# letao1991/EAD-GAN

Hardware: AMD Instinct MI355X
Metric: imgs/sec per G+D+E train step, CelebA 64x64 bs=128 (higher is better)
Workload: dtype bf16; 1 GPU; EAD-GAN CelebA 64x64x3 full train iteration (G adv + D + info/affine, 3 Adams), batch 128/GPU, hipGraph replay, data-parallel x1; per_gpu_batch=128, global_batch=128, parallelism=dp1

## Files before the change

### ead-gan_amd/csrc/img_conv.hip

```cpp

#include "eg_common.h"
#include "igemm_nt.h"

#ifndef EG_IMG_CONV_OCC
#define EG_IMG_CONV_OCC 3
#endif

struct ImgMfmaParams {
    const float* img[4];
    const float* gate[4];
    const void* wp;
    void* out;
    const float* bias;
    const float* sigma;
    int B, C, H, W;
    int act;
    float slope;
    int gate_act;
    float gate_slope;
    const void* stat_z;
    const float* stat_p[4];
    float* stat_out;
    int stat_act;
    float stat_slope;
};

constexpr int img_conv_occ(int N) { return N == 128 ? EG_IMG_CONV_OCC : (N == 64 ? 4 : 6); }
template <typename T, bool STAT, int N = 128>
__global__ __launch_bounds__(256, STAT ? 2 : img_conv_occ(N)) void conv_img_mfma_kernel(const ImgMfmaParams p, int ntiles) {
    static_assert(N == 128 || N == 64 || N == 32, "column tiles of 16, whole 64-byte chunks per pixel row");
    static_assert(!STAT || N == 128 || N == 64, "the statistics epilogue writes 2 N sums from 256 threads");
    constexpr int NJ = N / 16;
    constexpr int XS = 72, OS = N + 8;
    __shared__ __attribute__((aligned(16))) unsigned short s_in[4][6][XS];
    __shared__ __attribute__((aligned(16))) unsigned short s_out[4][16][OS];
    const int tid = threadIdx.x, lane = tid & 63, wave = tid >> 6;
    const int frow = lane & 15, fq = lane >> 4;
    const int OH = p.H >> 1, OW = p.W >> 1;
    const int gxn = OW >> 5, tpi = (OH >> 1) * gxn;
    const T* __restrict__ wp = reinterpret_cast<const T*>(p.wp);

    uint4 bf[2][NJ];
#pragma unroll
    for (int s = 0; s < 2; ++s)
#pragma unroll
        for (int j = 0; j < NJ; ++j) bf[s][j] = *reinterpret_cast<const uint4*>(wp + (size_t)(j * 16 + frow) * 64 + s * 32 + fq * 8);
    __shared__ __attribute__((aligned(16))) float s_bias[N];
    __shared__ __attribute__((aligned(16))) float s_red[STAT ? 4 * 2 * N : 4];
    if (tid < N) s_bias[tid] = p.bias ? p.bias[tid] : 0.f;
    __shared__ __attribute__((aligned(16))) float s_par[STAT ? 4 * N : 4];
    if constexpr (STAT) {
        if (tid < N) {
            const float mu = p.stat_p[0][tid], is = p.stat_p[1][tid], g = p.stat_p[2][tid], bb = p.stat_p[3][tid];
            const float P = __fmul_rn(g, is);
            s_par[tid] = mu; s_par[N + tid] = is; s_par[2 * N + tid] = P; s_par[3 * N + tid] = __fsub_rn(bb, __fmul_rn(mu, P));
        }
    }
    const EgGradFast sgf = eg_grad_fast(p.stat_act, p.stat_slope);
    const EgActFast af = eg_act_fast(p.act, p.slope);

    struct Slot { float4 v; float lo, hi; };
    auto fetch = [&](int tile, int e, Slot& sl) {
        sl.v = make_float4(0.f, 0.f, 0.f, 0.f); sl.lo = 0.f; sl.hi = 0.f;
        if (e >= 4 * 6 * 16 || tile >= ntiles) return;
        const int ib = tile / tpi, rem_t = tile - ib * tpi;
        const int tape = ib / p.B, b = ib - tape * p.B;
        const int gx = rem_t % gxn, oy0 = (rem_t / gxn) * 2;
        const int c = e / 96, rem = e - c * 96, r = rem >> 4, x4 = rem & 15;
        const int iy = 2 * oy0 - 1 + r, x0 = gx * 64;
        if (c >= p.C || iy < 0 || iy >= p.H) return;
        const size_t o = (((size_t)b * p.C + c) * p.H + iy) * p.W + x0 + x4 * 4;
        const float* __restrict__ img = p.img[tape];
        const float* __restrict__ gate = p.gate[tape];
        sl.v = *reinterpret_cast<const float4*>(img + o);
        if (x4 == 0 && x0 > 0) sl.lo = img[o - 1];
        if (x4 == 15 && x0 + 64 < p.W) sl.hi = img[o + 4];
        if (gate) {
            const float4 g = *reinterpret_cast<const float4*>(gate + o);
            sl.v.x *= eg_act_grad_from_out(g.x, p.gate_act, p.gate_slope); sl.v.y *= eg_act_grad_from_out(g.y, p.gate_act, p.gate_slope);
            sl.v.z *= eg_act_grad_from_out(g.z, p.gate_act, p.gate_slope); sl.v.w *= eg_act_grad_from_out(g.w, p.gate_act, p.gate_slope);
            if (x4 == 0 && x0 > 0) sl.lo *= eg_act_grad_from_out(gate[o - 1], p.gate_act, p.gate_slope);
            if (x4 == 15 && x0 + 64 < p.W) sl.hi *= eg_act_grad_from_out(gate[o + 4], p.gate_act, p.gate_slope);
        }
    };
    auto stage = [&](int e, const Slot& sl) {
        if (e >= 4 * 6 * 16) return;
        const int c = e / 96, rem = e - c * 96, r = rem >> 4, x4 = rem & 15;
        T h[4];
        Elt<T>::st(h + 0, sl.v.x); Elt<T>::st(h + 1, sl.v.y); Elt<T>::st(h + 2, sl.v.z); Elt<T>::st(h + 3, sl.v.w);
        unsigned short* row = &s_in[c][r][0];
        const unsigned short* hb = reinterpret_cast<const unsigned short*>(h);
        row[1 + x4 * 4] = hb[0];
        *reinterpret_cast<unsigned*>(row + 2 + x4 * 4) = (unsigned)hb[1] | ((unsigned)hb[2] << 16);
        row[4 + x4 * 4] = hb[3];
        if (x4 == 0) { T t; Elt<T>::st(&t, sl.lo); row[0] = *reinterpret_cast<const unsigned short*>(&t); }
        if (x4 == 15) { T t; Elt<T>::st(&t, sl.hi); row[65] = *reinterpret_cast<const unsigned short*>(&t); }
    };

    const int ry = wave >> 1, oxl = (wave & 1) * 16 + frow;
    const int r0 = 2 * ry + (fq & 1) * 2;
    auto ld8 = [&](int c, int r) {
        const unsigned* q = reinterpret_cast<const unsigned*>(&s_in[c][r][2 * oxl]);
        return make_uint2(q[0], q[1]);
    };
    T* __restrict__ out = reinterpret_cast<T*>(p.out);

    Slot s0, s1;
    int tile = blockIdx.x;
    fetch(tile, tid, s0); fetch(tile, tid + 256, s1);
    for (; tile < ntiles; tile += gridDim.x) {
        stage(tid, s0); stage(tid + 256, s1);
        __syncthreads();
        fetch(tile + gridDim.x, tid, s0); fetch(tile + gridDim.x, tid + 256, s1);
        const uint2 a00 = ld8(fq >> 1, r0), a01 = ld8(fq >> 1, r0 + 1);
        const uint2 a10 = ld8(2 + (fq >> 1), r0), a11 = ld8(2 + (fq >> 1), r0 + 1);
        const uint4 a0 = make_uint4(a00.x, a00.y, a01.x, a01.y), a1 = make_uint4(a10.x, a10.y, a11.x, a11.y);
        f32x4 acc[NJ];
#pragma unroll
        for (int j = 0; j < NJ; ++j) acc[j] = (f32x4){0.f, 0.f, 0.f, 0.f};
#pragma unroll
        for (int j = 0; j < NJ; ++j) mfma_step<T>(a0, bf[0][j], acc[j]);
#pragma unroll
        for (int j = 0; j < NJ; ++j) mfma_step<T>(a1, bf[1][j], acc[j]);
        const int ib = tile / tpi, rem_t = tile - ib * tpi;
        const int tape = ib / p.B;
        const int gx = rem_t % gxn, oy0 = (rem_t / gxn) * 2;
        const float inv_sigma = p.sigma ? 1.f / p.sigma[tape] : 1.f;
        const size_t pix0 = ((size_t)ib * OH + oy0 + ry) * OW + gx * 32 + (wave & 1) * 16;
#pragma unroll
        for (int j = 0; j < NJ; ++j) {
            T h[4];
            const float4 bv = *reinterpret_cast<const float4*>(&s_bias[j * 16 + fq * 4]);
            const float bj[4] = {bv.x, bv.y, bv.z, bv.w};
#pragma unroll
            for (int r = 0; r < 4; ++r) {
                float x = __fmul_rn(acc[j][r], inv_sigma);
                if (p.bias) x = __fadd_rn(x, bj[r]);
                x = af.special ? eg_act(x, p.act, p.slope) : eg_act_apply(x, af);
                Elt<T>::st(h + r, x);
            }
            if constexpr (STAT) {
                const uint2 zv = *reinterpret_cast<const uint2*>(reinterpret_cast<const T*>(p.stat_z) + (pix0 + frow) * N + j * 16 + fq * 4);
                const T* ze = reinterpret_cast<const T*>(&zv);
                float s1[4], s2[4];
                const int nb = j * 16 + fq * 4;
                const float4 vmu = *reinterpret_cast<const float4*>(&s_par[nb]), vis = *reinterpret_cast<const float4*>(&s_par[N + nb]);
                const float4 vp = *reinterpret_cast<const float4*>(&s_par[2 * N + nb]), vq = *reinterpret_cast<const float4*>(&s_par[3 * N + nb]);
                const float k_mu[4] = {vmu.x, vmu.y, vmu.z, vmu.w}, k_is[4] = {vis.x, vis.y, vis.z, vis.w};
                const float k_p[4] = {vp.x, vp.y, vp.z, vp.w}, k_q[4] = {vq.x, vq.y, vq.z, vq.w};
#pragma unroll
                for (int r = 0; r < 4; ++r) {
                    const float z = Elt<T>::ld(ze + r);
                    const float xh = (z - k_mu[r]) * k_is[r];
                    const float dy = Elt<T>::ld(h + r) * eg_grad_apply(fmaf(z, k_p[r], k_q[r]), sgf);
                    Elt<T>::st(h + r, dy);
                    s1[r] = dy;
                    s2[r] = dy * xh;
                }
#pragma unroll
                for (int r = 0; r < 4; ++r) {
                    s1[r] += eg_dpp<0xB1>(s1[r]); s1[r] += eg_dpp<0x4E>(s1[r]); s1[r] += eg_dpp<0x141>(s1[r]); s1[r] += eg_dpp<0x140>(s1[r]);
                    s2[r] += eg_dpp<0xB1>(s2[r]); s2[r] += eg_dpp<0x4E>(s2[r]); s2[r] += eg_dpp<0x141>(s2[r]); s2[r] += eg_dpp<0x140>(s2[r]);
                }
                if (frow == 0) {
                    *reinterpret_cast<float4*>(&s_red[(wave * 2 + 0) * N + j * 16 + fq * 4]) = make_float4(s1[0], s1[1], s1[2], s1[3]);
                    *reinterpret_cast<float4*>(&s_red[(wave * 2 + 1) * N + j * 16 + fq * 4]) = make_float4(s2[0], s2[1], s2[2], s2[3]);
                }
            }
            *reinterpret_cast<uint2*>(&s_out[wave][frow][j * 16 + fq * 4]) = *reinterpret_cast<const uint2*>(h);
        }
        __syncthreads();
        if constexpr (STAT) {
            if (tid < 2 * N) {
                const int which = tid / N, n = tid - which * N;
                const float t = ((s_red[(0 * 2 + which) * N + n] + s_red[(1 * 2 + which) * N + n]) + s_red[(2 * 2 + which) * N + n]) + s_red[(3 * 2 + which) * N + n];
                p.stat_out[((size_t)which * N + n) * ntiles + tile] = t;
            }
        }
        constexpr int CPR = N / 8, RPI = 64 / CPR;
#pragma unroll
        for (int it = 0; it < 16 / RPI; ++it) {
            const int row = it * RPI + lane / CPR, chunk = lane % CPR;
            const uint4 v = *reinterpret_cast<const uint4*>(&s_out[wave][row][chunk * 8]);
            *reinterpret_cast<uint4*>(out + (pix0 + row) * N + chunk * 8) = v;
        }
    }
}

extern "C" int eg_conv_img_mfma_stat_blocks(int B, int H, int W, int ntapes) { return (H / 4) * (W / 64) * B * ntapes; }

extern "C" int eg_conv_img_mfma_ok(int dtype, int C, int H, int W, int N, int k, int stride, int pad) {
    return dtype != EG_F32 && C >= 1 && C <= 4 && (N == 128 || N == 64 || N == 32) && k == 4 && stride == 2 && pad == 1 && H >= 4 && (H % 4) == 0 && (W % 64) == 0;
}

extern "C" int eg_conv_img_mfma_n(int dtype, const float* img0, const float* img1, const float* img2, const float* gate0, const float* gate1,
                                  const float* gate2, int ntapes, const void* wp, void* out, int B, int C, int H, int W, int N, const eg_epilogue* ep,
                                  int gate_act, float gate_slope, eg_stream_t s) {
    EG_REQUIRE(img0 && wp && out && ntapes >= 1 && ntapes <= 3 && B > 0, "eg_conv_img_mfma: bad argument");
    EG_REQUIRE(eg_conv_img_mfma_ok(dtype, C, H, W, N, 4, 2, 1), "eg_conv_img_mfma: 16-bit types, C <= 4, N = 32 / 64 / 128, H %% 4 == 0, W %% 64 == 0 only (use eg_im2col_img + eg_conv_fwd)");
    EG_REQUIRE((ntapes < 2 || img1) && (ntapes < 3 || img2), "eg_conv_img_mfma: one image pointer per tape");
    EG_REQUIRE(!ep || (!ep->mask && ep->out_mode == EG_OUT_NHWC && ep->bias_mod == 0 && (ep->stat_mode == EG_STAT_NONE || ep->stat_mode == EG_STAT_BN_BWD)),
               "eg_conv_img_mfma: unsupported epilogue field");
    const bool stat = ep && ep->stat_mode == EG_STAT_BN_BWD;
    EG_REQUIRE(!stat || N == 128 || N == 64, "eg_conv_img_mfma: EG_STAT_BN_BWD with 128 or 64 output channels only");
    EG_REQUIRE(!stat || (ep->stat_out && ep->stat_aux && ep->stat_p0 && ep->stat_p1 && ep->stat_p2 && ep->stat_p3), "eg_conv_img_mfma: EG_STAT_BN_BWD needs stat_out, stat_aux (z) and stat_p0..p3");
    ImgMfmaParams p;
    memset(&p, 0, sizeof(p));
    p.img[0] = img0; p.img[1] = img1; p.img[2] = img2;
    p.gate[0] = gate0; p.gate[1] = gate1; p.gate[2] = gate2;
    p.wp = wp; p.out = out; p.B = B; p.C = C; p.H = H; p.W = W;
    p.bias = ep ? ep->bias : nullptr;
    p.sigma = ep ? ep->sigma : nullptr;
    p.act = ep ? ep->act : EG_ACT_NONE;
    p.slope = ep ? ep->slope : 0.f;
    p.gate_act = gate_act; p.gate_slope = gate_slope;
    if (stat) {
        p.stat_z = ep->stat_aux; p.stat_out = ep->stat_out; p.stat_act = ep->stat_act; p.stat_slope = ep->stat_slope;
        p.stat_p[0] = ep->stat_p0; p.stat_p[1] = ep->stat_p1; p.stat_p[2] = ep->stat_p2; p.stat_p[3] = ep->stat_p3;
    }
    const int ntiles = (H / 4) * (W / 64) * B * ntapes;
    const int wgs_n = N == 128 ? 256 * EG_IMG_CONV_OCC : 256 * img_conv_occ(N);
    const dim3 grid(ntiles < wgs_n ? ntiles : wgs_n);
    if (stat) {
        const dim3 gs(ntiles < 512 ? ntiles : 512);
        if (N == 64) {
            if (dtype == EG_F16) hipLaunchKernelGGL((conv_img_mfma_kernel<f16_t, true, 64>), gs, dim3(256), 0, (hipStream_t)s, p, ntiles);
            else hipLaunchKernelGGL((conv_img_mfma_kernel<bf16_t, true, 64>), gs, dim3(256), 0, (hipStream_t)s, p, ntiles);
        } else if (dtype == EG_F16) hipLaunchKernelGGL((conv_img_mfma_kernel<f16_t, true>), gs, dim3(256), 0, (hipStream_t)s, p, ntiles);
        else hipLaunchKernelGGL((conv_img_mfma_kernel<bf16_t, true>), gs, dim3(256), 0, (hipStream_t)s, p, ntiles);
    } else if (N == 128) {
        if (dtype == EG_F16) hipLaunchKernelGGL((conv_img_mfma_kernel<f16_t, false>), grid, dim3(256), 0, (hipStream_t)s, p, ntiles);
        else hipLaunchKernelGGL((conv_img_mfma_kernel<bf16_t, false>), grid, dim3(256), 0, (hipStream_t)s, p, ntiles);
    } else if (N == 64) {
        if (dtype == EG_F16) hipLaunchKernelGGL((conv_img_mfma_kernel<f16_t, false, 64>), grid, dim3(256), 0, (hipStream_t)s, p, ntiles);
        else hipLaunchKernelGGL((conv_img_mfma_kernel<bf16_t, false, 64>), grid, dim3(256), 0, (hipStream_t)s, p, ntiles);
    } else {
        if (dtype == EG_F16) hipLaunchKernelGGL((conv_img_mfma_kernel<f16_t, false, 32>), grid, dim3(256), 0, (hipStream_t)s, p, ntiles);
        else hipLaunchKernelGGL((conv_img_mfma_kernel<bf16_t, false, 32>), grid, dim3(256), 0, (hipStream_t)s, p, ntiles);
    }
    EG_LAUNCH_CHECK();
    return 0;
}

extern "C" int eg_conv_img_mfma(int dtype, const float* img0, const float* img1, const float* img2, const float* gate0, const float* gate1,
                                const float* gate2, int ntapes, const void* wp, void* out, int B, int C, int H, int W, const eg_epilogue* ep,
                                int gate_act, float gate_slope, eg_stream_t s) {
    return eg_conv_img_mfma_n(dtype, img0, img1, img2, gate0, gate1, gate2, ntapes, wp, out, B, C, H, W, 128, ep, gate_act, gate_slope, s);
}

struct ImgTParams {
    const void* a;
    const void* wp;
    const float* bias;
    float* out;
    int B, C, Hin, Win;
    int act;
    float slope;
};

template <typename T, int R, int K = 128>
__global__ __launch_bounds__(256) void convt_img_mfma_kernel(const ImgTParams p) {
    constexpr int KS = K / 32;
    constexpr int WMAX = 32, NP = 56;
    __shared__ __attribute__((aligned(16))) unsigned short s_cols[(R + 2) * WMAX * NP];
    const int tid = threadIdx.x, lane = tid & 63, wave = tid >> 6;
    const int frow = lane & 15, fq = lane >> 4;
    const int nblk = p.Hin / R, b = blockIdx.x / nblk, r0 = (blockIdx.x % nblk) * R;
    const int ncol = 16 * p.C;
    const T* __restrict__ wp = reinterpret_cast<const T*>(p.wp);
    const T* __restrict__ a = reinterpret_cast<const T*>(p.a) + (size_t)b * p.Hin * p.Win * K;

    uint4 bf[KS][3];
#pragma unroll
    for (int s = 0; s < KS; ++s)
#pragma unroll
        for (int j = 0; j < 3; ++j) {
            const int n = j * 16 + frow;
            bf[s][j] = n < ncol ? *reinterpret_cast<const uint4*>(wp + (size_t)n * K + s * 32 + fq * 8) : make_uint4(0, 0, 0, 0);
        }
    const int npix = (R + 2) * p.Win, ngrp = npix / 16;
    auto fetch = [&](int g, uint4 (&af)[KS]) {
        const int pl = g * 16 + frow;
        const int iy = r0 - 1 + pl / p.Win, ix = pl % p.Win;
        const bool ok = g < ngrp && iy >= 0 && iy < p.Hin;
#pragma unroll
        for (int s = 0; s < KS; ++s)
            af[s] = ok ? *reinterpret_cast<const uint4*>(a + ((size_t)iy * p.Win + ix) * K + s * 32 + fq * 8) : make_uint4(0, 0, 0, 0);
    };
    auto compute = [&](int g, const uint4 (&af)[KS]) {
        const int pl = g * 16 + frow;
        f32x4 acc[3];
#pragma unroll
        for (int j = 0; j < 3; ++j) acc[j] = (f32x4){0.f, 0.f, 0.f, 0.f};
#pragma unroll
        for (int s = 0; s < KS; ++s)
#pragma unroll
            for (int j = 0; j < 3; ++j) mfma_step<T>(af[s], bf[s][j], acc[j]);
#pragma unroll
        for (int j = 0; j < 3; ++j) {
            T h[4];
#pragma unroll
            for (int r = 0; r < 4; ++r) Elt<T>::st(h + r, __fmul_rn(acc[j][r], 1.f));
            *reinterpret_cast<uint2*>(&s_cols[(size_t)pl * NP + j * 16 + fq * 4]) = *reinterpret_cast<const uint2*>(h);
        }
    };
    uint4 fa[KS], fb[KS];
    fetch(wave, fa);
    for (int g = wave; g < ngrp; g += 8) {
        fetch(g + 4, fb);
        compute(g, fa);
        if (g + 4 < ngrp) {
            fetch(g + 8, fa);
            compute(g + 4, fb);
        }
    }
    __syncthreads();
    const int OH = 2 * p.Hin, OW = 2 * p.Win;
    const T* __restrict__ cols = reinterpret_cast<const T*>(s_cols);
    for (int o = tid; o < 2 * R * OW; o += 256) {
        const int ox = o % OW, oy = 2 * r0 + o / OW;
        float acc[3];
#pragma unroll
        for (int c = 0; c < 3; ++c) acc[c] = (p.bias && c < p.C) ? p.bias[c] : 0.f;
        for (int kh = (oy + 1) & 1; kh < 4; kh += 2) {
            const int iy = (oy + 1 - kh) >> 1;
            if (iy < 0 || iy >= p.Hin) continue;
            for (int kw = (ox + 1) & 1; kw < 4; kw += 2) {
                const int ix = (ox + 1 - kw) >> 1;
                if (ix < 0 || ix >= p.Win) continue;
                const T* src = cols + (size_t)((iy - (r0 - 1)) * p.Win + ix) * NP + (kh * 4 + kw) * p.C;
#pragma unroll
                for (int c = 0; c < 3; ++c)
                    if (c < p.C) acc[c] += Elt<T>::ld(src + c);
            }
        }
#pragma unroll
        for (int c = 0; c < 3; ++c)
            if (c < p.C) p.out[(((size_t)b * p.C + c) * OH + oy) * OW + ox] = eg_act(acc[c], p.act, p.slope);
    }
}

extern "C" int eg_convt_img_mfma_ok(int dtype, int C, int Hin, int Win, int K, int k, int stride, int pad) {
    return dtype != EG_F32 && C >= 1 && C <= 3 && (K == 128 || K == 64) && k == 4 && stride == 2 && pad == 1 && Hin >= 16 && (Hin % 16) == 0 && (Win == 16 || Win == 32);
}

extern "C" int eg_convt_img_mfma_k(int dtype, const void* a, const void* wp, const float* bias, float* out, int B, int C, int Hin, int Win, int K, int act,
                                   float slope, eg_stream_t s) {
    EG_REQUIRE(a && wp && out && B > 0, "eg_convt_img_mfma: bad argument");
    EG_REQUIRE(eg_convt_img_mfma_ok(dtype, C, Hin, Win, K, 4, 2, 1), "eg_convt_img_mfma: 16-bit types, C <= 3, K = 64 / 128, Hin %% 16 == 0, Win 16 or 32 only (use eg_conv_fwd + eg_col2im_img)");
    ImgTParams p;
    memset(&p, 0, sizeof(p));
    p.a = a; p.wp = wp; p.bias = bias; p.out = out; p.B = B; p.C = C; p.Hin = Hin; p.Win = Win; p.act = act; p.slope = slope;
    hipStream_t st = (hipStream_t)s;
    if (K == 64) {
        const dim3 grid(B * (Hin / 8));
        if (dtype == EG_F16) hipLaunchKernelGGL((convt_img_mfma_kernel<f16_t, 8, 64>), grid, dim3(256), 0, st, p);
        else hipLaunchKernelGGL((convt_img_mfma_kernel<bf16_t, 8, 64>), grid, dim3(256), 0, st, p);
        EG_LAUNCH_CHECK();
        return 0;
    }
    const dim3 grid(B * (Hin / 8));
    if (dtype == EG_F16) hipLaunchKernelGGL((convt_img_mfma_kernel<f16_t, 8>), grid, dim3(256), 0, st, p);
    else hipLaunchKernelGGL((convt_img_mfma_kernel<bf16_t, 8>), grid, dim3(256), 0, st, p);
    EG_LAUNCH_CHECK();
    return 0;
}
extern "C" int eg_convt_img_mfma(int dtype, const void* a, const void* wp, const float* bias, float* out, int B, int C, int Hin, int Win, int act,
                                 float slope, eg_stream_t s) {
    return eg_convt_img_mfma_k(dtype, a, wp, bias, out, B, C, Hin, Win, 128, act, slope, s);
}

struct ImgWgradParams {
    const float* img[4];
    const void* P;
    float* slab;
    int B, C, ntiles;
};

template <typename T, int N>
__global__ __launch_bounds__(256) void wgrad_img_kernel(const ImgWgradParams p) {
    constexpr int H = 64, W = 64, OW = 32, XS = 72;
    constexpr int PP = N + 8, PX = 72;
    constexpr int NI = N / 16;
    __shared__ __attribute__((aligned(16))) unsigned short s_in[4][10][XS];
    __shared__ __attribute__((aligned(16))) unsigned short s_px[128 * PP + 128 * PX];
    unsigned short* s_p = s_px;
    unsigned short* s_x = s_px + 128 * PP;
    static_assert(4 * N * 16 * sizeof(float) <= (128 * PP + 128 * PX) * sizeof(unsigned short), "the reduction scratch lies over the operand tiles");
    float (*s_red)[N][16] = reinterpret_cast<float (*)[N][16]>(s_px);
    const int tid = threadIdx.x, lane = tid & 63, wave = tid >> 6;
    const int g = lane >> 4, li = lane & 15, q = li >> 2, pc = li & 3;
    const int kc = p.C * 16, nj = p.C;
    const T* __restrict__ P = reinterpret_cast<const T*>(p.P);
    for (int i = tid; i < 4 * 10 * XS; i += 256) (&s_in[0][0][0])[i] = 0;
    for (int i = tid; i < 128 * PX; i += 256) s_x[i] = 0;
    f32x4 acc[NI][4];
#pragma unroll
    for (int i = 0; i < NI; ++i)
#pragma unroll
        for (int j = 0; j < 4; ++j) acc[i][j] = (f32x4){0.f, 0.f, 0.f, 0.f};
    typedef __attribute__((address_space(3))) s16x4* lds_s16x4;
    auto tr2 = [&](const unsigned short* base, int pitch, int row, int blk) {
        const s16x4 lo = __builtin_amdgcn_ds_read_tr16_b64_v4i16((lds_s16x4)(base + (row + q) * pitch + blk * 16 + pc * 4));
        const s16x4 hi = __builtin_amdgcn_ds_read_tr16_b64_v4i16((lds_s16x4)(base + (row + 4 + q) * pitch + blk * 16 + pc * 4));
        return make_uint4(((uint32_t)(uint16_t)lo[0]) | ((uint32_t)(uint16_t)lo[1] << 16), ((uint32_t)(uint16_t)lo[2]) | ((uint32_t)(uint16_t)lo[3] << 16),
                          ((uint32_t)(uint16_t)hi[0]) | ((uint32_t)(uint16_t)hi[1] << 16), ((uint32_t)(uint16_t)hi[2]) | ((uint32_t)(uint16_t)hi[3] << 16));
    };
    for (int tile = blockIdx.x; tile < p.ntiles; tile += gridDim.x) {
        const int ib = tile >> 3, oy0 = (tile & 7) * 4;
        const int tape = ib / p.B, b = ib - tape * p.B;
        const float* __restrict__ img = p.img[tape] + (size_t)b * p.C * H * W;
        __syncthreads();
        for (int e = tid; e < p.C * 10 * 16; e += 256) {
            const int c = e / 160, rem = e - c * 160, r = rem >> 4, x4 = rem & 15;
            const int iy = 2 * oy0 - 1 + r;
            float4 v = make_float4(0.f, 0.f, 0.f, 0.f);
            if (iy >= 0 && iy < H) v = *reinterpret_cast<const float4*>(img + ((size_t)c * H + iy) * W + x4 * 4);
            T h[4];
            Elt<T>::st(h + 0, v.x); Elt<T>::st(h + 1, v.y); Elt<T>::st(h + 2, v.z); Elt<T>::st(h + 3, v.w);
            const unsigned short* hb = reinterpret_cast<const unsigned short*>(h);
            unsigned short* row = &s_in[c][r][1 + x4 * 4];
            row[0] = hb[0]; row[1] = hb[1]; row[2] = hb[2]; row[3] = hb[3];
        }
        const T* __restrict__ Pt = P + ((size_t)ib * 1024 + (size_t)oy0 * OW) * N;
        for (int e = tid; e < 128 * (N / 8); e += 256) {
            const int row = e / (N / 8), ch = e - row * (N / 8);
            *reinterpret_cast<uint4*>(&s_p[row * PP + ch * 8]) = *reinterpret_cast<const uint4*>(Pt + (size_t)row * N + ch * 8);
        }
        __syncthreads();
        for (int e = tid; e < 128 * kc; e += 256) {
            const int pix = e / kc, k = e - pix * kc;
            const int c = k >> 4, ky = (k >> 2) & 3, kx = k & 3;
            s_x[pix * PX + k] = s_in[c][2 * (pix >> 5) + ky][2 * (pix & 31) + kx];
        }
        __syncthreads();
        const int kb = wave * 32 + 8 * g;
        uint4 af[NI], bfr[4];
#pragma unroll
        for (int i = 0; i < NI; ++i) af[i] = tr2(s_p, PP, kb, i);
#pragma unroll
        for (int j = 0; j < 4; ++j)
            if (j < nj) bfr[j] = tr2(s_x, PX, kb, j);
#pragma unroll
        for (int i = 0; i < NI; ++i)
#pragma unroll
            for (int j = 0; j < 4; ++j)
                if (j < nj) {
                    if constexpr (std::is_same<T, f16_t>::value)
                        acc[i][j] = __builtin_amdgcn_mfma_f32_16x16x32_f16(__builtin_bit_cast(f16x8_t, af[i]), __builtin_bit_cast(f16x8_t, bfr[j]), acc[i][j], 0, 0, 0);
                    else
                        acc[i][j] = __builtin_amdgcn_mfma_f32_16x16x32_bf16(__builtin_bit_cast(bf16x8_t, af[i]), __builtin_bit_cast(bf16x8_t, bfr[j]), acc[i][j], 0, 0, 0);
                }
    }
    float* slab = p.slab + (size_t)blockIdx.x * N * kc;
    for (int j = 0; j < nj; ++j) {
        __syncthreads();
#pragma unroll
        for (int i = 0; i < NI; ++i)
#pragma unroll
            for (int r = 0; r < 4; ++r) {
                float v = 0.f;
#pragma unroll
                for (int jj = 0; jj < 4; ++jj)
                    if (jj == j) v = acc[i][jj][r];
                s_red[wave][i * 16 + g * 4 + r][li] = v;
            }
        __syncthreads();
        for (int e = tid; e < N * 16; e += 256) {
            const int n = e >> 4, k = e & 15;
            slab[(size_t)n * kc + j * 16 + k] = ((s_red[0][n][k] + s_red[1][n][k]) + s_red[2][n][k]) + s_red[3][n][k];
        }
    }
}

extern "C" int eg_wgrad_img_ok(int dtype, int C, int H, int W, int N, int k, int stride, int pad) {
    return dtype != EG_F32 && C >= 1 && C <= 4 && (N == 32 || N == 64 || N == 128) && k == 4 && stride == 2 && pad == 1 && H == 64 && W == 64;
}
extern "C" int eg_wgrad_img_splits_n(int images, int N) {
    const long long tiles = (long long)images * 8, cap = N >= 128 ? 256 : 1024;
    return (int)(tiles < cap ? tiles : cap);
}
extern "C" int eg_wgrad_img_splits(int images) { return eg_wgrad_img_splits_n(images, 32); }
extern "C" int eg_wgrad_img(int dtype, const float* img0, const float* img1, const float* img2, int ntapes, const void* P, float* slab, int B, int C,
                            int H, int W, int N, int* nsplit_out, eg_stream_t s) {
    EG_REQUIRE(img0 && P && slab && nsplit_out && ntapes >= 1 && ntapes <= 3 && B > 0, "eg_wgrad_img: bad argument");
    EG_REQUIRE((ntapes < 2 || img1) && (ntapes < 3 || img2), "eg_wgrad_img: one image pointer per tape");
    EG_REQUIRE(eg_wgrad_img_ok(dtype, C, H, W, N, 4, 2, 1), "eg_wgrad_img: 16-bit types, C <= 4, N = 32 / 64 / 128, 64 x 64 images, 4x4 / stride 2 / pad 1 only (use eg_im2col_img + eg_conv_wgrad)");
    ImgWgradParams p;
    memset(&p, 0, sizeof(p));
    p.img[0] = img0; p.img[1] = img1; p.img[2] = img2;
    p.P = P; p.slab = slab; p.B = B; p.C = C; p.ntiles = ntapes * B * 8;
    const int grid = eg_wgrad_img_splits_n(ntapes * B, N);
    hipStream_t st = (hipStream_t)s;
    if (N == 128) {
        if (dtype == EG_F16) hipLaunchKernelGGL((wgrad_img_kernel<f16_t, 128>), dim3(grid), dim3(256), 0, st, p);
        else hipLaunchKernelGGL((wgrad_img_kernel<bf16_t, 128>), dim3(grid), dim3(256), 0, st, p);
    } else if (N == 32) {
        if (dtype == EG_F16) hipLaunchKernelGGL((wgrad_img_kernel<f16_t, 32>), dim3(grid), dim3(256), 0, st, p);
        else hipLaunchKernelGGL((wgrad_img_kernel<bf16_t, 32>), dim3(grid), dim3(256), 0, st, p);
    } else {
        if (dtype == EG_F16) hipLaunchKernelGGL((wgrad_img_kernel<f16_t, 64>), dim3(grid), dim3(256), 0, st, p);
        else hipLaunchKernelGGL((wgrad_img_kernel<bf16_t, 64>), dim3(grid), dim3(256), 0, st, p);
    }
    *nsplit_out = grid;
    EG_LAUNCH_CHECK();
    return 0;
}
```

Before: 30010 imgs/s.

## Double-buffer image conv tiles, prefetch BN inputs, specialize gated kernel variants

The image-input MFMA conv kernel now double-buffers its input staging tile, which removes the second per-tile __syncthreads. Per-tile BN statistics stores are deferred by one iteration, and the z tensor for the BN-backward epilogue is prefetched into registers and staged through shared memory. Gate loads are split from the gate-derivative math, which is now done at staging time with a tanh fast path. A compile-time GATE template parameter and per-variant occupancy bounds are added. Grid sizing now follows the per-variant occupancy, and inverse sigma is hoisted out of the loop. This costs more LDS and registers, and occupancy drops for the gated and stat variants.

After: 30280 imgs/s (median of 6 runs). Within noise of the previous version (+0.9%).

```diff
diff --git a/ead-gan_amd/csrc/img_conv.hip b/ead-gan_amd/csrc/img_conv.hip
--- a/ead-gan_amd/csrc/img_conv.hip
+++ b/ead-gan_amd/csrc/img_conv.hip
@@ -1,10 +1,6 @@
 
 #include "eg_common.h"
 #include "igemm_nt.h"
-
-#ifndef EG_IMG_CONV_OCC
-#define EG_IMG_CONV_OCC 3
-#endif
 
 struct ImgMfmaParams {
     const float* img[4];
@@ -25,14 +21,18 @@
     float stat_slope;
 };
 
-constexpr int img_conv_occ(int N) { return N == 128 ? EG_IMG_CONV_OCC : (N == 64 ? 4 : 6); }
-template <typename T, bool STAT, int N = 128>
-__global__ __launch_bounds__(256, STAT ? 2 : img_conv_occ(N)) void conv_img_mfma_kernel(const ImgMfmaParams p, int ntiles) {
+constexpr int img_conv_occ(int N, bool stat, bool gated) {
+    return N == 128 ? (stat || gated ? 2 : 3) : (N == 64 ? (stat ? 3 : 4) : (gated ? 5 : 6));
+}
+
+template <typename T, bool STAT, int N, bool GATE>
+__global__ __launch_bounds__(256, img_conv_occ(N, STAT, GATE)) void conv_img_mfma_kernel(const ImgMfmaParams p, int ntiles) {
     static_assert(N == 128 || N == 64 || N == 32, "column tiles of 16, whole 64-byte chunks per pixel row");
     static_assert(!STAT || N == 128 || N == 64, "the statistics epilogue writes 2 N sums from 256 threads");
     constexpr int NJ = N / 16;
     constexpr int XS = 72, OS = N + 8;
-    __shared__ __attribute__((aligned(16))) unsigned short s_in[4][6][XS];
+    constexpr int CPR = N / 8, RPI = 64 / CPR, NIT = 16 / RPI;
+    __shared__ __attribute__((aligned(16))) unsigned short s_in[2][4][6][XS];
     __shared__ __attribute__((aligned(16))) unsigned short s_out[4][16][OS];
     const int tid = threadIdx.x, lane = tid & 63, wave = tid >> 6;
     const int frow = lane & 15, fq = lane >> 4;
@@ -46,7 +46,7 @@
 #pragma unroll
         for (int j = 0; j < NJ; ++j) bf[s][j] = *reinterpret_cast<const uint4*>(wp + (size_t)(j * 16 + frow) * 64 + s * 32 + fq * 8);
     __shared__ __attribute__((aligned(16))) float s_bias[N];
-    __shared__ __attribute__((aligned(16))) float s_red[STAT ? 4 * 2 * N : 4];
+    __shared__ __attribute__((aligned(16))) float s_red[STAT ? 2 * 4 * 2 * N : 4];
     if (tid < N) s_bias[tid] = p.bias ? p.bias[tid] : 0.f;
     __shared__ __attribute__((aligned(16))) float s_par[STAT ? 4 * N : 4];
     if constexpr (STAT) {
@@ -58,37 +58,69 @@
     }
     const EgGradFast sgf = eg_grad_fast(p.stat_act, p.stat_slope);
     const EgActFast af = eg_act_fast(p.act, p.slope);
-
-    struct Slot { float4 v; float lo, hi; };
+    float isg[3];
+#pragma unroll
+    for (int t = 0; t < 3; ++t) isg[t] = (p.sigma && p.img[t]) ? 1.f / p.sigma[t] : 1.f;
+
+    struct TileAt { int ib, tape, b, gx, oy0; };
+    auto decode = [&](int tile) {
+        TileAt t;
+        t.ib = tile / tpi;
+        const int rem_t = tile - t.ib * tpi;
+        t.tape = t.ib / p.B; t.b = t.ib - t.tape * p.B;
+        t.gx = rem_t % gxn; t.oy0 = (rem_t / gxn) * 2;
+        return t;
+    };
+    const int ry = wave >> 1, oxl = (wave & 1) * 16 + frow;
+    auto first_pixel = [&](const TileAt& t) { return ((size_t)t.ib * OH + t.oy0 + ry) * OW + t.gx * 32 + (wave & 1) * 16; };
+
+    enum { HAVE = 1, HAVE_LO = 2, HAVE_HI = 4, GATED = 8 };
+    struct Slot { float4 v, g; float lo, hi, glo, ghi; int fl; };
     auto fetch = [&](int tile, int e, Slot& sl) {
-        sl.v = make_float4(0.f, 0.f, 0.f, 0.f); sl.lo = 0.f; sl.hi = 0.f;
+        sl.v = make_float4(0.f, 0.f, 0.f, 0.f); sl.lo = 0.f; sl.hi = 0.f; sl.fl = 0;
+        if constexpr (GATE) { sl.g = make_float4(0.f, 0.f, 0.f, 0.f); sl.glo = 0.f; sl.ghi = 0.f; }
         if (e >= 4 * 6 * 16 || tile >= ntiles) return;
-        const int ib = tile / tpi, rem_t = tile - ib * tpi;
-        const int tape = ib / p.B, b = ib - tape * p.B;
-        const int gx = rem_t % gxn, oy0 = (rem_t / gxn) * 2;
+        const TileAt t = decode(tile);
         const int c = e / 96, rem = e - c * 96, r = rem >> 4, x4 = rem & 15;
-        const int iy = 2 * oy0 - 1 + r, x0 = gx * 64;
+        const int iy = 2 * t.oy0 - 1 + r, x0 = t.gx * 64;
         if (c >= p.C || iy < 0 || iy >= p.H) return;
-        const size_t o = (((size_t)b * p.C + c) * p.H + iy) * p.W + x0 + x4 * 4;
-        const float* __restrict__ img = p.img[tape];
-        const float* __restrict__ gate = p.gate[tape];
+        const size_t o = (((size_t)t.b * p.C + c) * p.H + iy) * p.W + x0 + x4 * 4;
+        const float* __restrict__ img = p.img[t.tape];
         sl.v = *reinterpret_cast<const float4*>(img + o);
-        if (x4 == 0 && x0 > 0) sl.lo = img[o - 1];
-        if (x4 == 15 && x0 + 64 < p.W) sl.hi = img[o + 4];
-        if (gate) {
-            const float4 g = *reinterpret_cast<const float4*>(gate + o);
-            sl.v.x *= eg_act_grad_from_out(g.x, p.gate_act, p.gate_slope); sl.v.y *= eg_act_grad_from_out(g.y, p.gate_act, p.gate_slope);
-            sl.v.z *= eg_act_grad_from_out(g.z, p.gate_act, p.gate_slope); sl.v.w *= eg_act_grad_from_out(g.w, p.gate_act, p.gate_slope);
-            if (x4 == 0 && x0 > 0) sl.lo *= eg_act_grad_from_out(gate[o - 1], p.gate_act, p.gate_slope);
-            if (x4 == 15 && x0 + 64 < p.W) sl.hi *= eg_act_grad_from_out(gate[o + 4], p.gate_act, p.gate_slope);
-        }
-    };
-    auto stage = [&](int e, const Slot& sl) {
+        sl.fl = HAVE;
+        if (x4 == 0 && x0 > 0) { sl.lo = img[o - 1]; sl.fl |= HAVE_LO; }
+        if (x4 == 15 && x0 + 64 < p.W) { sl.hi = img[o + 4]; sl.fl |= HAVE_HI; }
+        if constexpr (GATE) {
+            const float* __restrict__ gate = p.gate[t.tape];
+            if (gate) {
+                sl.g = *reinterpret_cast<const float4*>(gate + o);
+                if (sl.fl & HAVE_LO) sl.glo = gate[o - 1];
+                if (sl.fl & HAVE_HI) sl.ghi = gate[o + 4];
+                sl.fl |= GATED;
+            }
+        }
+    };
+    auto stage = [&](int buf, int e, Slot& sl) {
         if (e >= 4 * 6 * 16) return;
+        if constexpr (GATE) {
+            if (sl.fl & GATED) {
+                auto mul = [&](auto is_tanh) {
+                    auto dact = [&](float a) {
+                        if constexpr (decltype(is_tanh)::value) return fmaf(-a, a, 1.f);
+                        else return eg_act_grad_from_out(a, p.gate_act, p.gate_slope);
+                    };
+                    sl.v.x *= dact(sl.g.x); sl.v.y *= dact(sl.g.y); sl.v.z *= dact(sl.g.z); sl.v.w *= dact(sl.g.w);
+                    if (sl.fl & HAVE_LO) sl.lo *= dact(sl.glo);
+                    if (sl.fl & HAVE_HI) sl.hi *= dact(sl.ghi);
+                };
+                if (p.gate_act == EG_ACT_TANH) mul(std::true_type{});
+                else mul(std::false_type{});
+            }
+        }
         const int c = e / 96, rem = e - c * 96, r = rem >> 4, x4 = rem & 15;
         T h[4];
         Elt<T>::st(h + 0, sl.v.x); Elt<T>::st(h + 1, sl.v.y); Elt<T>::st(h + 2, sl.v.z); Elt<T>::st(h + 3, sl.v.w);
-        unsigned short* row = &s_in[c][r][0];
+        unsigned short* row = &s_in[buf][c][r][0];
         const unsigned short* hb = reinterpret_cast<const unsigned short*>(h);
         row[1 + x4 * 4] = hb[0];
         *reinterpret_cast<unsigned*>(row + 2 + x4 * 4) = (unsigned)hb[1] | ((unsigned)hb[2] << 16);
@@ -96,24 +128,52 @@
         if (x4 == 0) { T t; Elt<T>::st(&t, sl.lo); row[0] = *reinterpret_cast<const unsigned short*>(&t); }
         if (x4 == 15) { T t; Elt<T>::st(&t, sl.hi); row[65] = *reinterpret_cast<const unsigned short*>(&t); }
     };
-
-    const int ry = wave >> 1, oxl = (wave & 1) * 16 + frow;
+    const int drow = lane / CPR, dchunk = lane % CPR;
+    typedef __attribute__((ext_vector_type(4))) unsigned u32x4;
+    constexpr int NZ = STAT ? NIT : 1;
+    u32x4 zr[NZ];
+#pragma unroll
+    for (int it = 0; it < NZ; ++it) zr[it] = (u32x4){0u, 0u, 0u, 0u};
+    auto fetch_z = [&](int tile, u32x4 (&zq)[NZ]) {
+        if (tile >= ntiles) return;
+        const T* __restrict__ z = reinterpret_cast<const T*>(p.stat_z) + first_pixel(decode(tile)) * N;
+#pragma unroll
+        for (int it = 0; it < NZ; ++it) zq[it] = *reinterpret_cast<const u32x4*>(z + (size_t)(it * RPI + drow) * N + dchunk * 8);
+    };
+    auto store_sums = [&](int par, int tile) {
+        if (tid < 2 * N) {
+            const int which = tid / N, n = tid - which * N;
+            const float* red = &s_red[par * 4 * 2 * N];
+            const float t = ((red[(0 * 2 + which) * N + n] + red[(1 * 2 + which) * N + n]) + red[(2 * 2 + which) * N + n]) + red[(3 * 2 + which) * N + n];
+            p.stat_out[((size_t)which * N + n) * ntiles + tile] = t;
+        }
+    };
+
     const int r0 = 2 * ry + (fq & 1) * 2;
-    auto ld8 = [&](int c, int r) {
-        const unsigned* q = reinterpret_cast<const unsigned*>(&s_in[c][r][2 * oxl]);
+    auto ld8 = [&](int buf, int c, int r) {
+        const unsigned* q = reinterpret_cast<const unsigned*>(&s_in[buf][c][r][2 * oxl]);
         return make_uint2(q[0], q[1]);
     };
     T* __restrict__ out = reinterpret_cast<T*>(p.out);
 
     Slot s0, s1;
-    int tile = blockIdx.x;
+    int tile = blockIdx.x, buf = 0, prev = -1;
     fetch(tile, tid, s0); fetch(tile, tid + 256, s1);
-    for (; tile < ntiles; tile += gridDim.x) {
-        stage(tid, s0); stage(tid + 256, s1);
+    if constexpr (STAT) fetch_z(tile, zr);
+    for (; tile < ntiles; prev = tile, tile += gridDim.x, buf ^= 1) {
+        stage(buf, tid, s0); stage(buf, tid + 256, s1);
+        if constexpr (STAT) {
+#pragma unroll
+            for (int it = 0; it < NIT; ++it) *reinterpret_cast<u32x4*>(&s_out[wave][it * RPI + drow][dchunk * 8]) = zr[it];
+        }
         __syncthreads();
         fetch(tile + gridDim.x, tid, s0); fetch(tile + gridDim.x, tid + 256, s1);
-        const uint2 a00 = ld8(fq >> 1, r0), a01 = ld8(fq >> 1, r0 + 1);
-        const uint2 a10 = ld8(2 + (fq >> 1), r0), a11 = ld8(2 + (fq >> 1), r0 + 1);
+        if constexpr (STAT) {
+            fetch_z(tile + gridDim.x, zr);
+            if (prev >= 0) store_sums(buf ^ 1, prev);
+        }
+        const uint2 a00 = ld8(buf, fq >> 1, r0), a01 = ld8(buf, fq >> 1, r0 + 1);
+        const uint2 a10 = ld8(buf, 2 + (fq >> 1), r0), a11 = ld8(buf, 2 + (fq >> 1), r0 + 1);
         const uint4 a0 = make_uint4(a00.x, a00.y, a01.x, a01.y), a1 = make_uint4(a10.x, a10.y, a11.x, a11.y);
         f32x4 acc[NJ];
 #pragma unroll
@@ -122,68 +182,66 @@
         for (int j = 0; j < NJ; ++j) mfma_step<T>(a0, bf[0][j], acc[j]);
 #pragma unroll
         for (int j = 0; j < NJ; ++j) mfma_step<T>(a1, bf[1][j], acc[j]);
-        const int ib = tile / tpi, rem_t = tile - ib * tpi;
-        const int tape = ib / p.B;
-        const int gx = rem_t % gxn, oy0 = (rem_t / gxn) * 2;
-        const float inv_sigma = p.sigma ? 1.f / p.sigma[tape] : 1.f;
-        const size_t pix0 = ((size_t)ib * OH + oy0 + ry) * OW + gx * 32 + (wave & 1) * 16;
-#pragma unroll
-        for (int j = 0; j < NJ; ++j) {
-            T h[4];
-            const float4 bv = *reinterpret_cast<const float4*>(&s_bias[j * 16 + fq * 4]);
-            const float bj[4] = {bv.x, bv.y, bv.z, bv.w};
-#pragma unroll
-            for (int r = 0; r < 4; ++r) {
-                float x = __fmul_rn(acc[j][r], inv_sigma);
-                if (p.bias) x = __fadd_rn(x, bj[r]);
-                x = af.special ? eg_act(x, p.act, p.slope) : eg_act_apply(x, af);
-                Elt<T>::st(h + r, x);
+        const TileAt at = decode(tile);
+        const float inv_sigma = at.tape == 0 ? isg[0] : (at.tape == 1 ? isg[1] : isg[2]);
+        const size_t pix0 = first_pixel(at);
+        float* red = &s_red[STAT ? buf * 4 * 2 * N : 0];
+        eg_if_fast(af.special, [&](auto fast) {
+    #pragma unroll
+            for (int j = 0; j < NJ; ++j) {
+                T h[4];
+                const float4 bv = *reinterpret_cast<const float4*>(&s_bias[j * 16 + fq * 4]);
+                const float bj[4] = {bv.x, bv.y, bv.z, bv.w};
+    #pragma unroll
+                for (int r = 0; r < 4; ++r) {
+                    float x = __fmul_rn(acc[j][r], inv_sigma);
+                    if (p.bias) x = __fadd_rn(x, bj[r]);
+                    if constexpr (decltype(fast)::value) x = eg_act_apply(x, af);
+                    else { x = eg_act(x, p.act, p.slope); __builtin_amdgcn_sched_barrier(0); }
+                    Elt<T>::st(h + r, x);
+                }
+                if constexpr (STAT) {
+                    const uint2 zv = *reinterpret_cast<const uint2*>(&s_out[wave][frow][j * 16 + fq * 4]);
+                    const T* ze = reinterpret_cast<const T*>(&zv);
+                    float s1[4], s2[4];
+                    const int nb = j * 16 + fq * 4;
+                    const float4 vmu = *reinterpret_cast<const float4*>(&s_par[nb]), vis = *reinterpret_cast<const float4*>(&s_par[N + nb]);
+                    const float4 vp = *reinterpret_cast<const float4*>(&s_par[2 * N + nb]), vq = *reinterpret_cast<const float4*>(&s_par[3 * N + nb]);
+                    const float k_mu[4] = {vmu.x, vmu.y, vmu.z, vmu.w}, k_is[4] = {vis.x, vis.y, vis.z, vis.w};
+                    const float k_p[4] = {vp.x, vp.y, vp.z, vp.w}, k_q[4] = {vq.x, vq.y, vq.z, vq.w};
+    #pragma unroll
+                    for (int r = 0; r < 4; ++r) {
+                        const float z = Elt<T>::ld(ze + r);
+                        const float xh = (z - k_mu[r]) * k_is[r];
+                        const float dy = Elt<T>::ld(h + r) * eg_grad_apply(fmaf(z, k_p[r], k_q[r]), sgf);
+                        Elt<T>::st(h + r, dy);
+                        s1[r] = dy;
+                        s2[r] = dy * xh;
+                    }
+    #pragma unroll
+                    for (int r = 0; r < 4; ++r) {
+                        s1[r] += eg_dpp<0xB1>(s1[r]); s1[r] += eg_dpp<0x4E>(s1[r]); s1[r] += eg_dpp<0x141>(s1[r]); s1[r] += eg_dpp<0x140>(s1[r]);
+                        s2[r] += eg_dpp<0xB1>(s2[r]); s2[r] += eg_dpp<0x4E>(s2[r]); s2[r] += eg_dpp<0x141>(s2[r]); s2[r] += eg_dpp<0x140>(s2[r]);
+                    }
+                    if (frow == 0) {
+                        *reinterpret_cast<float4*>(&red[(wave * 2 + 0) * N + j * 16 + fq * 4]) = make_float4(s1[0], s1[1], s1[2], s1[3]);
+                        *reinterpret_cast<float4*>(&red[(wave * 2 + 1) * N + j * 16 + fq * 4]) = make_float4(s2[0], s2[1], s2[2], s2[3]);
+                    }
+                }
+                *reinterpret_cast<uint2*>(&s_out[wave][frow][j * 16 + fq * 4]) = *reinterpret_cast<const uint2*>(h);
             }
-            if constexpr (STAT) {
-                const uint2 zv = *reinterpret_cast<const uint2*>(reinterpret_cast<const T*>(p.stat_z) + (pix0 + frow) * N + j * 16 + fq * 4);
-                const T* ze = reinterpret_cast<const T*>(&zv);
-                float s1[4], s2[4];
-                const int nb = j * 16 + fq * 4;
-                const float4 vmu = *reinterpret_cast<const float4*>(&s_par[nb]), vis = *reinterpret_cast<const float4*>(&s_par[N + nb]);
-                const float4 vp = *reinterpret_cast<const float4*>(&s_par[2 * N + nb]), vq = *reinterpret_cast<const float4*>(&s_par[3 * N + nb]);
-                const float k_mu[4] = {vmu.x, vmu.y, vmu.z, vmu.w}, k_is[4] = {vis.x, vis.y, vis.z, vis.w};
-                const float k_p[4] = {vp.x, vp.y, vp.z, vp.w}, k_q[4] = {vq.x, vq.y, vq.z, vq.w};
-#pragma unroll
-                for (int r = 0; r < 4; ++r) {
-                    const float z = Elt<T>::ld(ze + r);
-                    const float xh = (z - k_mu[r]) * k_is[r];
-                    const float dy = Elt<T>::ld(h + r) * eg_grad_apply(fmaf(z, k_p[r], k_q[r]), sgf);
-                    Elt<T>::st(h + r, dy);
-                    s1[r] = dy;
-                    s2[r] = dy * xh;
-                }
-#pragma unroll
-                for (int r = 0; r < 4; ++r) {
-                    s1[r] += eg_dpp<0xB1>(s1[r]); s1[r] += eg_dpp<0x4E>(s1[r]); s1[r] += eg_dpp<0x141>(s1[r]); s1[r] += eg_dpp<0x140>(s1[r]);
-                    s2[r] += eg_dpp<0xB1>(s2[r]); s2[r] += eg_dpp<0x4E>(s2[r]); s2[r] += eg_dpp<0x141>(s2[r]); s2[r] += eg_dpp<0x140>(s2[r]);
-                }
-                if (frow == 0) {
-                    *reinterpret_cast<float4*>(&s_red[(wave * 2 + 0) * N + j * 16 + fq * 4]) = make_float4(s1[0], s1[1], s1[2], s1[3]);
-                    *reinterpret_cast<float4*>(&s_red[(wave * 2 + 1) * N + j * 16 + fq * 4]) = make_float4(s2[0], s2[1], s2[2], s2[3]);
-                }
-            }
-            *reinterpret_cast<uint2*>(&s_out[wave][frow][j * 16 + fq * 4]) = *reinterpret_cast<const uint2*>(h);
-        }
-        __syncthreads();
-        if constexpr (STAT) {
-            if (tid < 2 * N) {
-                const int which = tid / N, n = tid - which * N;
-                const float t = ((s_red[(0 * 2 + which) * N + n] + s_red[(1 * 2 + which) * N + n]) + s_red[(2 * 2 + which) * N + n]) + s_red[(3 * 2 + which) * N + n];
-                p.stat_out[((size_t)which * N + n) * ntiles + tile] = t;
-            }
-        }
-        constexpr int CPR = N / 8, RPI = 64 / CPR;
-#pragma unroll
-        for (int it = 0; it < 16 / RPI; ++it) {
-            const int row = it * RPI + lane / CPR, chunk = lane % CPR;
-            const uint4 v = *reinterpret_cast<const uint4*>(&s_out[wave][row][chunk * 8]);
-            *reinterpret_cast<uint4*>(out + (pix0 + row) * N + chunk * 8) = v;
-        }
+        });
+        __builtin_amdgcn_wave_barrier();
+#pragma unroll
+        for (int it = 0; it < NIT; ++it) {
+            const int row = it * RPI + drow;
+            const uint4 v = *reinterpret_cast<const uint4*>(&s_out[wave][row][dchunk * 8]);
+            *reinterpret_cast<uint4*>(out + (pix0 + row) * N + dchunk * 8) = v;
+        }
+    }
+    if constexpr (STAT) {
+        __syncthreads();
+        store_sums(buf ^ 1, prev);
     }
 }
 
@@ -219,25 +277,21 @@
         p.stat_p[0] = ep->stat_p0; p.stat_p[1] = ep->stat_p1; p.stat_p[2] = ep->stat_p2; p.stat_p[3] = ep->stat_p3;
     }
     const int ntiles = (H / 4) * (W / 64) * B * ntapes;
-    const int wgs_n = N == 128 ? 256 * EG_IMG_CONV_OCC : 256 * img_conv_occ(N);
-    const dim3 grid(ntiles < wgs_n ? ntiles : wgs_n);
-    if (stat) {
-        const dim3 gs(ntiles < 512 ? ntiles : 512);
-        if (N == 64) {
-            if (dtype == EG_F16) hipLaunchKernelGGL((conv_img_mfma_kernel<f16_t, true, 64>), gs, dim3(256), 0, (hipStream_t)s, p, ntiles);
-            else hipLaunchKernelGGL((conv_img_mfma_kernel<bf16_t, true, 64>), gs, dim3(256), 0, (hipStream_t)s, p, ntiles);
-        } else if (dtype == EG_F16) hipLaunchKernelGGL((conv_img_mfma_kernel<f16_t, true>), gs, dim3(256), 0, (hipStream_t)s, p, ntiles);
-        else hipLaunchKernelGGL((conv_img_mfma_kernel<bf16_t, true>), gs, dim3(256), 0, (hipStream_t)s, p, ntiles);
-    } else if (N == 128) {
-        if (dtype == EG_F16) hipLaunchKernelGGL((conv_img_mfma_kernel<f16_t, false>), grid, dim3(256), 0, (hipStream_t)s, p, ntiles);
-        else hipLaunchKernelGGL((conv_img_mfma_kernel<bf16_t, false>), grid, dim3(256), 0, (hipStream_t)s, p, ntiles);
-    } else if (N == 64) {
-        if (dtype == EG_F16) hipLaunchKernelGGL((conv_img_mfma_kernel<f16_t, false, 64>), grid, dim3(256), 0, (hipStream_t)s, p, ntiles);
-        else hipLaunchKernelGGL((conv_img_mfma_kernel<bf16_t, false, 64>), grid, dim3(256), 0, (hipStream_t)s, p, ntiles);
-    } else {
-        if (dtype == EG_F16) hipLaunchKernelGGL((conv_img_mfma_kernel<f16_t, false, 32>), grid, dim3(256), 0, (hipStream_t)s, p, ntiles);
-        else hipLaunchKernelGGL((conv_img_mfma_kernel<bf16_t, false, 32>), grid, dim3(256), 0, (hipStream_t)s, p, ntiles);
-    }
+    const bool gated = gate0 || gate1 || gate2;
+    auto go = [&](auto kernel, int occ) {
+        const int wgs = 256 * occ;
+        hipLaunchKernelGGL(kernel, dim3(ntiles < wgs ? ntiles : wgs), dim3(256), 0, (hipStream_t)s, p, ntiles);
+    };
+    auto pick = [&](auto t) {
+        using T = decltype(t);
+        if (stat && N == 128) gated ? go(conv_img_mfma_kernel<T, true, 128, true>, img_conv_occ(128, true, true)) : go(conv_img_mfma_kernel<T, true, 128, false>, img_conv_occ(128, true, false));
+        else if (stat) gated ? go(conv_img_mfma_kernel<T, true, 64, true>, img_conv_occ(64, true, true)) : go(conv_img_mfma_kernel<T, true, 64, false>, img_conv_occ(64, true, false));
+        else if (N == 128) gated ? go(conv_img_mfma_kernel<T, false, 128, true>, img_conv_occ(128, false, true)) : go(conv_img_mfma_kernel<T, false, 128, false>, img_conv_occ(128, false, false));
+        else if (N == 64) gated ? go(conv_img_mfma_kernel<T, false, 64, true>, img_conv_occ(64, false, true)) : go(conv_img_mfma_kernel<T, false, 64, false>, img_conv_occ(64, false, false));
+        else gated ? go(conv_img_mfma_kernel<T, false, 32, true>, img_conv_occ(32, false, true)) : go(conv_img_mfma_kernel<T, false, 32, false>, img_conv_occ(32, false, false));
+    };
+    if (dtype == EG_F16) pick(f16_t{});
+    else pick(bf16_t{});
     EG_LAUNCH_CHECK();
     return 0;
 }
```
